# jdeschut/tunempc

Measured on AMD Instinct MI355X. Metric: stage-Hessian convexifications/sec at (nx+nu)=32, p=64, higher is better.
Workload: dtype f64

## Files before the change

include/tunempc_hip.h:

```cpp
#ifndef TUNEMPC_HIP_H
#define TUNEMPC_HIP_H

#include <stdint.h>

#ifdef __cplusplus
extern "C" {
#endif

#define TMPC_OK 0
#define TMPC_E_ARG (-1)
#define TMPC_E_UNSUPPORTED (-2)
#define TMPC_E_NOMEM (-3)
#define TMPC_E_HIP (-4)
#define TMPC_E_NODEVICE (-5)
#define TMPC_E_NOCONV (-6)

#define TMPC_STATUS_OPTIMAL 0
#define TMPC_STATUS_FEASIBLE 1
#define TMPC_STATUS_INFEASIBLE 2

#define TMPC_FLAG_NO_MFMA 1
#define TMPC_FLAG_PROFILE 2
#define TMPC_FLAG_FAST_EXIT 4

// ... 13 lines not shown
uint64_t tmpc_workspace_bytes_con(int chunk, int p, int nx, int mb, int ng, int nc);
int tmpc_create_con(tmpc_handle** out, int chunk, int p, int nx, int mb, int ng, int nc);
int tmpc_destroy(tmpc_handle* h);
int tmpc_get_chunk(tmpc_handle* h);

int tmpc_set_options(tmpc_handle* h, double tol, double center_tol, int max_iter, int center_iter, int flags);

#define TMPC_TUNE_CHORD_STEP 1
#define TMPC_TUNE_SMALL_BLOCKS 2
#define TMPC_TUNE_EIG_PRETEST 3
#define TMPC_TUNE_FUSE_FWD 4
#define TMPC_TUNE_GRAPH 5
#define TMPC_TUNE_PERSISTENT 7
#define TMPC_TUNE_LOWP_SWITCH 8
#define TMPC_LOWP_SWITCH_DEFAULT 1e-5
int tmpc_set_tuning(tmpc_handle* h, int key, double value);
int tmpc_create_ex(tmpc_handle** out, int chunk, int p, int nx, int mb, int ng, int nc, int step3, int lanes);

int tmpc_set_tight(tmpc_handle* h, int enable, double tight_tol);

int tmpc_convexify_batch_host(tmpc_handle* h, int nb, const double* A, const double* B, const double* H,
                              double* Hc, double* dHc, double* P, double* alpha, double* beta, double* kappa,
                              int32_t* status, int32_t* iters, double* info);
int tmpc_convexify_batch_device(tmpc_handle* h, int nb, const double* dA, const double* dB, const double* dH,
                                double* dHc_out, double* ddHc_out, double* dP_out, double* d_alpha, double* d_beta,
                                double* d_kappa, int32_t* d_status, int32_t* d_iters, double* d_info, void* stream);

int tmpc_convexify_eq_batch_host(tmpc_handle* h, int nb, const double* A, const double* B, const double* H, const double* G,
                                 double* Hc, double* dHc, double* P, double* Fg, double* alpha, double* beta, double* kappa,
                                 int32_t* status, int32_t* iters, double* info);
// ... 56 lines not shown
```

tunempc_amd/_lib.py:

```python
import ctypes as C
import os

import numpy as np

_HERE = os.path.dirname(os.path.abspath(__file__))
_LIB = None

INFO_STRIDE = 16
FLAG_NO_MFMA = 1
FLAG_PROFILE = 2
FLAG_FAST_EXIT = 4
STATUS_NAMES = {0: 'Optimal', 1: 'Feasible', 2: 'Infeasible'}

ARROW_LD = 32
EXPORTS = [
    'tmpc_device_count', 'tmpc_workspace_bytes', 'tmpc_workspace_bytes_eq', 'tmpc_workspace_bytes_con',
    'tmpc_create', 'tmpc_create_eq', 'tmpc_create_con', 'tmpc_destroy', 'tmpc_get_chunk', 'tmpc_set_options', 'tmpc_set_tight', 'tmpc_set_tuning', 'tmpc_create_ex',
    'tmpc_convexify_batch_host', 'tmpc_convexify_batch_device', 'tmpc_convexify_eq_batch_host', 'tmpc_convexify_step2_batch_host',
    'tmpc_convexify_con_batch_device', 'tmpc_workspace_bytes_step3', 'tmpc_create_step3', 'tmpc_convexify_step3_batch_host', 'tmpc_workspace_bytes_step3_con', 'tmpc_create_step3_con', 'tmpc_convexify_step3_con_batch_host', 'tmpc_convexify_step3_batch_device', 'tmpc_convexify_step3_con_batch_device', 'tmpc_supplement_batch_host', 'tmpc_supplement_terms_batch_host',
    'tmpc_tracking_reference_host', 'tmpc_eig_scan_host', 'tmpc_get_profile', 'tmpc_get_trace', 'tmpc_get_dual_host', 'tmpc_get_dual_con_host', 'tmpc_pack_sensitivities_host', 'tmpc_eig_clip_host',
    'tmpc_last_error', 'tmpc_version',
]
DEBUG_EXPORTS = [
    'tmpc_debug_gemm_nt', 'tmpc_debug_block_solve', 'tmpc_debug_cr_schedule', 'tmpc_debug_get_multipliers', 'tmpc_debug_get_array',
# ... 148 lines not shown
            _check(self.lib, self.lib.tmpc_create_step3_con(C.byref(self._h), int(chunk), self.p, self.nx, self.mb, self.ng, self.nc), 'tmpc_create_step3_con')
        elif self.step3:
            _check(self.lib, self.lib.tmpc_create_step3(C.byref(self._h), int(chunk), self.p, self.nx, self.mb), 'tmpc_create_step3')
        else:
            _check(self.lib, self.lib.tmpc_create_con(C.byref(self._h), int(chunk), self.p, self.nx, self.mb, self.ng, self.nc), 'tmpc_create_con')
        self.chunk = int(self.lib.tmpc_get_chunk(self._h))
        self.flags = int(flags)
        self.set_options(tol, center_tol, max_iter, center_iter, flags)

    def set_options(self, tol=None, center_tol=None, max_iter=None, center_iter=None, flags=None):
        if flags is not None:
            self.flags = int(flags)
        _check(self.lib, self.lib.tmpc_set_options(self._h, float(tol or 0.0), float(center_tol or 0.0),
                                                   int(max_iter or 0), int(center_iter or 0), self.flags), 'tmpc_set_options')

    def set_tuning(self, chord_step=None, small_blocks=None, eig_pretest=None, fuse_fwd=None, graph=None, persistent=None, lowp_switch=None):
        for key, v in ((1, chord_step), (2, small_blocks), (3, eig_pretest), (4, fuse_fwd), (5, graph), (7, persistent), (8, lowp_switch)):
            if v is not None:
                _check(self.lib, self.lib.tmpc_set_tuning(self._h, key, float(v)), 'tmpc_set_tuning')

    def set_tight(self, enable=True, tight_tol=None):
        _check(self.lib, self.lib.tmpc_set_tight(self._h, 1 if enable else 0, float(tight_tol or 0.0)), 'tmpc_set_tight')

    def close(self):
        if getattr(self, '_h', None) is not None and self._h.value:
            self.lib.tmpc_destroy(self._h)
            self._h = C.c_void_p()

    def __del__(self):
        try:
            self.close()
        except Exception:
# ... 336 lines not shown
```

tunempc_amd/csrc/tmpc_api.hip:

```cpp
#include <hip/hip_runtime.h>
#include <stdio.h>
#include <stdlib.h>
#include <new>
#include <string.h>
#include <algorithm>
#include <chrono>
#include <thread>
#include <mutex>
#include <condition_variable>
#include <functional>
#include <unistd.h>
#include <vector>

#include <string>
#include <unordered_map>

#include "../../include/tunempc_hip.h"
#include "../../include/tunempc_hip_debug.h"
#include "tmpc_common.h"
#include "tmpc_small.h"
#include "tmpc_stage.h"
#include "tmpc_schur.h"
#include "tmpc_factor.h"
#include "tmpc_cr.h"
// ... 89 lines not shown

struct tmpc_handle {
  Dims dm;
  int chunk;
  int nlanes;
  Opts opt;
  int flags;
  Lane lane[MAXL];
  void* slab;
  size_t slab_bytes;
  hipEvent_t ev_in;
  int device;
  CrSched sched;
  int* d_sched;
  int rs, mt;
  int tune_small, tune_pretest, tune_fuse, tune_graph, tune_persist;
  void* dd_slab;
  size_t dd_bytes;
  int tight;
  double tight_tol;
};

static int cr_upload(const CrSched& sc, int** out) {
  std::vector<int> flat(sc.elim);
  flat.insert(flat.end(), sc.upd.begin(), sc.upd.end());
  flat.insert(flat.end(), sc.orient.begin(), sc.orient.end());
  *out = nullptr;
  if (hipMalloc(out, flat.size() * sizeof(int)) != hipSuccess) return TMPC_E_NOMEM;
  if (hipMemcpy(*out, flat.data(), flat.size() * sizeof(int), hipMemcpyHostToDevice) != hipSuccess) { hipFree(*out); *out = nullptr; return TMPC_E_HIP; }
  return TMPC_OK;
}
// ... 289 lines not shown
static int set_lds_attrs(int device) {
  static bool done[64] = {false};
  if (device >= 0 && device < 64 && done[device]) return TMPC_OK;
  const int big = 160 * 1024;
  HIPCHK(hipFuncSetAttribute((const void*)k_stage_pre<256>, hipFuncAttributeMaxDynamicSharedMemorySize, big - 4096));
  HIPCHK(hipFuncSetAttribute((const void*)k_stage_rhs<256>, hipFuncAttributeMaxDynamicSharedMemorySize, big - 4096));
  HIPCHK(hipFuncSetAttribute((const void*)k_stage_dir<256>, hipFuncAttributeMaxDynamicSharedMemorySize, big - 4096));
  HIPCHK(hipFuncSetAttribute((const void*)k_final_stage, hipFuncAttributeMaxDynamicSharedMemorySize, big));
  HIPCHK(hipFuncSetAttribute((const void*)k_schur<0>, hipFuncAttributeMaxDynamicSharedMemorySize, big));
  HIPCHK(hipFuncSetAttribute((const void*)k_schur<1>, hipFuncAttributeMaxDynamicSharedMemorySize, big));
  HIPCHK(hipFuncSetAttribute((const void*)k_cr_potrf<true>, hipFuncAttributeMaxDynamicSharedMemorySize, big));
  HIPCHK(hipFuncSetAttribute((const void*)k_cr_potrf<false>, hipFuncAttributeMaxDynamicSharedMemorySize, big));
  HIPCHK(hipFuncSetAttribute((const void*)k_cr_trsm<true, 2>, hipFuncAttributeMaxDynamicSharedMemorySize, big));
  HIPCHK(hipFuncSetAttribute((const void*)k_cr_trsm<false, 2>, hipFuncAttributeMaxDynamicSharedMemorySize, big));
  HIPCHK(hipFuncSetAttribute((const void*)k_cr_trsm_dma, hipFuncAttributeMaxDynamicSharedMemorySize, big));
  HIPCHK(hipFuncSetAttribute((const void*)k_cr_potrf_dma, hipFuncAttributeMaxDynamicSharedMemorySize, big));
  HIPCHK(hipFuncSetAttribute((const void*)k_cr_update<true, 2>, hipFuncAttributeMaxDynamicSharedMemorySize, big));
  HIPCHK(hipFuncSetAttribute((const void*)k_cr_update<false, 2>, hipFuncAttributeMaxDynamicSharedMemorySize, big));
  HIPCHK(hipFuncSetAttribute((const void*)k_cr_fwd_diag, hipFuncAttributeMaxDynamicSharedMemorySize, big));
  HIPCHK(hipFuncSetAttribute((const void*)k_cr_fwd_off, hipFuncAttributeMaxDynamicSharedMemorySize, big));
  HIPCHK(hipFuncSetAttribute((const void*)k_cr_bwd, hipFuncAttributeMaxDynamicSharedMemorySize, big));
  HIPCHK(hipFuncSetAttribute((const void*)k_cr_small_solve, hipFuncAttributeMaxDynamicSharedMemorySize, big));
  HIPCHK(hipFuncSetAttribute((const void*)k_cr_small_factor, hipFuncAttributeMaxDynamicSharedMemorySize, big));
  HIPCHK(hipFuncSetAttribute((const void*)k_ipm_small, hipFuncAttributeMaxDynamicSharedMemorySize, big));
  HIPCHK(hipFuncSetAttribute((const void*)k_debug_gemm<true>, hipFuncAttributeMaxDynamicSharedMemorySize, big));
  HIPCHK(hipFuncSetAttribute((const void*)k_debug_gemm<false>, hipFuncAttributeMaxDynamicSharedMemorySize, big));
  HIPCHK(hipFuncSetAttribute((const void*)k_supplement, hipFuncAttributeMaxDynamicSharedMemorySize, big));
  HIPCHK(hipFuncSetAttribute((const void*)k_phi_pre<false, false>, hipFuncAttributeMaxDynamicSharedMemorySize, big));
  HIPCHK(hipFuncSetAttribute((const void*)k_phi_pre<false, true>, hipFuncAttributeMaxDynamicSharedMemorySize, big));
  HIPCHK(hipFuncSetAttribute((const void*)k_phi_pre<true, false>, hipFuncAttributeMaxDynamicSharedMemorySize, big));
// ... 12 lines not shown
  HIPCHK(hipFuncSetAttribute((const void*)k_dd_fwd_off, hipFuncAttributeMaxDynamicSharedMemorySize, big));
  HIPCHK(hipFuncSetAttribute((const void*)k_dd_bwd, hipFuncAttributeMaxDynamicSharedMemorySize, big));
  HIPCHK(hipFuncSetAttribute((const void*)k_dd_images, hipFuncAttributeMaxDynamicSharedMemorySize, big));
  HIPCHK(hipFuncSetAttribute((const void*)k_dd_schur<0>, hipFuncAttributeMaxDynamicSharedMemorySize, big));
  HIPCHK(hipFuncSetAttribute((const void*)k_dd_schur<1>, hipFuncAttributeMaxDynamicSharedMemorySize, big));
  HIPCHK(hipFuncSetAttribute((const void*)k_dd_schur<0, true>, hipFuncAttributeMaxDynamicSharedMemorySize, big));
  HIPCHK(hipFuncSetAttribute((const void*)k_dd_schur<1, true>, hipFuncAttributeMaxDynamicSharedMemorySize, big));
  HIPCHK(hipFuncSetAttribute((const void*)k_dd_polish_pre, hipFuncAttributeMaxDynamicSharedMemorySize, big - 4096));
  HIPCHK(hipFuncSetAttribute((const void*)k_polish_step, hipFuncAttributeMaxDynamicSharedMemorySize, big - 4096));
  if (device >= 0 && device < 64) done[device] = true;
  return TMPC_OK;
}

static unsigned cr_grid(long items) { return (unsigned)((items + 7) / 8 * 8); }
constexpr int DF_NO_SMALL = 2;
constexpr int DF_LOWP = 8;
constexpr int DF_NO_DMA = 4;

static bool cr_small_levels(const Dims& dm, const CrSched& sc, CrLevs* out) {
  if ((dm.flags & DF_NO_SMALL) || dm.dp != 16 || (dm.flags & 1) || dm.p > CRS_PMAX || (int)sc.lev.size() > CRS_MAXLEV) return false;
  if (out) {
    out->n = (int)sc.lev.size();
    for (int l = 0; l < out->n; ++l) { out->v[4 * l] = sc.lev[l].eoff; out->v[4 * l + 1] = sc.lev[l].nelim; out->v[4 * l + 2] = sc.lev[l].uoff; out->v[4 * l + 3] = sc.lev[l].nupd; }
  }
  return true;
}

static void cr_factor(const WS& w, const Dims& dm, const CrSched& sc, const int* d_sched, const int* alist, int count, hipStream_t st,
                      int rs_opt, int mt_opt, std::vector<hipEvent_t>* kev = nullptr, int* nkev = nullptr, int fuse_fwd1 = 0, int nlowp = 0) {
  const CrDev cd = cr_dev(sc, d_sched, alist);
  int ke = 0;
// ... 26 lines not shown
      hipLaunchKernelGGL(k_cr_potrf_dma, dim3(cr_grid((long)count * lv.nelim)), dim3(256), (size_t)potrf_dma_lds_doubles() * sizeof(double), st, w, dm, cd, lv.eoff, lv.nelim, count);
    else if (mf) hipLaunchKernelGGL(k_cr_potrf<true>, dim3(cr_grid((long)count * lv.nelim)), dim3(256), factor_lds(), st, w, dm, cd, lv.eoff, lv.nelim, count);
    else hipLaunchKernelGGL(k_cr_potrf<false>, dim3(cr_grid((long)count * lv.nelim)), dim3(256), factor_lds(), st, w, dm, cd, lv.eoff, lv.nelim, count);
    mark(0);
    if (fuse_fwd1) hipLaunchKernelGGL(k_cr_fwd_diag, dim3(cr_grid((long)count * lv.nelim)), dim3(256), solve_lds(dm), st, w, dm, cd, lv.eoff, lv.nelim, count, 1);
    if (lv.nupd == 0) { mark(1); mark(1); mark(2); mark(2); mark(3); mark(3); continue; }
    const long work64 = (long)count * lv.nelim * 2 * nt64;
    const int rs = rs_opt > 0 ? rs_opt : (work64 >= 16384 ? 128 : 64);
    const int mt = mt_opt > 0 ? mt_opt : 64;
    const int nstrip = (dm.dp + rs - 1) / rs, nm = (dm.dp + mt - 1) / mt;
    const long it_trsm = (long)count * lv.nelim * 2 * nstrip;
    const long it_upd = (long)count * ((long)lv.nupd * (nm * (nm + 1) / 2) + (long)lv.nelim * nm * nm);
    mark(1);
    if (mf && use_dma && dm.nt <= TRR_NT) {
      const size_t trsm_lds = (size_t)trd_lds_doubles() * sizeof(double);
      hipLaunchKernelGGL(k_cr_trsm_dma, dim3(cr_grid((long)count * lv.nelim * 2 * nt64)), dim3(256), trsm_lds, st, w, dm, cd, lv.eoff, lv.nelim, count);
    }
    else if (mf) hipLaunchKernelGGL((k_cr_trsm<true, 2>), dim3(cr_grid(it_trsm)), dim3(256), factor_lds(), st, w, dm, cd, lv.eoff, lv.nelim, count, rs);
    else hipLaunchKernelGGL((k_cr_trsm<false, 2>), dim3(cr_grid(it_trsm)), dim3(256), factor_lds(), st, w, dm, cd, lv.eoff, lv.nelim, count, rs);
    mark(1); mark(2);
    if (mf && use_dma) {
      const int nm64 = (dm.dp + 63) / 64;
      const long it_dma = (long)count * ((long)lv.nupd * (nm64 * (nm64 + 1) / 2) + (long)lv.nelim * nm64 * nm64);
      if (nlowp < count)
        hipLaunchKernelGGL(k_cr_update_dma, dim3(cr_grid(it_dma)), dim3(256), (size_t)dma_lds_doubles<UPD_DMA_DEPTH>() * sizeof(double), st, w, dm, cd, lv.eoff, lv.nelim, lv.uoff, lv.nupd, count, fuse_fwd1);
      mark(2); mark(3);
      if (nlowp > 0)
        hipLaunchKernelGGL(k_cr_update_dma_f32, dim3(cr_grid(it_dma)), dim3(256), (size_t)UPD_DMA_DEPTH * DMA_SLAB * sizeof(double), st, w, dm, cd, lv.eoff, lv.nelim, lv.uoff, lv.nupd, count);
      mark(3);
    }
    else if (mf) { hipLaunchKernelGGL((k_cr_update<true, 2>), dim3(cr_grid(it_upd)), dim3(256), factor_lds(), st, w, dm, cd, lv.eoff, lv.nelim, lv.uoff, lv.nupd, count, mt); mark(2); mark(3); mark(3); }
// ... 95 lines not shown
    if (hipMalloc(&ln->big_scr, (size_t)h->dm.B * dm.p * BIG_SCR * dm.n * dm.n * sizeof(double)) != hipSuccess) { snprintf(g_err, sizeof(g_err), "hipMalloc of the generic-stage scratch failed"); return TMPC_E_NOMEM; }
    ln->ws.bscr = (double*)ln->big_scr;
  }
  WS wall = ln->ws;
  wall.A = dA; wall.Bm = dB; wall.H = dH; wall.G = dG; wall.ncnt = dncnt; wall.rho = rho;
  wall.cr_orient = h->d_sched + h->sched.elim.size() + h->sched.upd.size();
  WS w = wall;
  w.A = nullptr; w.Bm = nullptr; w.H = nullptr;
  int* alist = wall.alist;
  int* flist = wall.flist;
  wall.alist = nullptr;
  Opts o = h->opt;
  o.tight = 0; o.tight_tol = 0.0;
  o.fast_exit = (h->flags & TMPC_FLAG_FAST_EXIT) ? 1 : 0;
  if ((h->flags & (TMPC_FLAG_NO_MFMA | TMPC_DEBUG_FLAG_NO_DMA)) || !w.O32 || t3 || dm.dp <= 64 || dm.nt > TRR_NT) o.lowp_switch = 0.0;
  if (o.lowp_switch > 0.0) {
    dm.flags |= DF_LOWP;
    if (ln->o32_dp != 0 && ln->o32_dp != dm.dp) HIPCHK(hipMemsetAsync(w.O32, 0, 2 * (size_t)h->dm.B * h->dm.p * h->dm.dp * ((h->dm.dp + 31) & ~31) * sizeof(float), st));
    ln->o32_dp = dm.dp;
  }
  WS wf = w; wf.alist = flist;
  const int BPall = nb * dm.p;
  const bool prof = (h->flags & TMPC_FLAG_PROFILE) != 0;
  bool use_graph = h->tune_graph && dm.dp <= 64 && !(h->flags & (TMPC_FLAG_PROFILE | TMPC_DEBUG_FLAG_STOP_ASSEMBLED)) && st == ln->st;
  const int reg_max = (h->flags & TMPC_DEBUG_FLAG_NO_LIFT) ? 0 : REG_MAX;
  HIPCHK(hipMemsetAsync(w.active, 0, 5 * sizeof(int), st));
  HIPCHK(hipMemsetAsync(w.trace, 0, (size_t)nb * TRACE_LEN * TRACE_W * sizeof(double), st));
  const size_t big_lds = (size_t)BIG_EIG_LDS * sizeof(double);
  if (big) hipLaunchKernelGGL(kb_init_stage, dim3(BPall), dim3(256), big_lds, st, wall, dm);
  else hipLaunchKernelGGL(k_init_stage, dim3(BPall), dim3(64), slots_bytes(2), st, wall, dm);
  {
    WS wi = wall; wi.alist = alist;
    hipLaunchKernelGGL(k_init_prob, dim3(nb), dim3(64), 0, st, wi, dm);
  }
  hipLaunchKernelGGL(k_init_state, dim3(BPall), dim3(64), 0, st, wall, dm);
  if (eq) hipLaunchKernelGGL(k_phi_init, dim3(BPall), dim3(64), 0, st, wall, dm);
  if (t3) hipLaunchKernelGGL(k_t3_init, dim3(BPall), dim3(64), 0, st, wall, dm);
  int cnt[5] = {0, 0, 0, 0, 0};
  HIPCHK(hipMemcpyAsync(cnt, w.active, 5 * sizeof(int), hipMemcpyDeviceToHost, st));
  HIPCHK(hipStreamSynchronize(st));
  int active = cnt[0], nfac = cnt[0], nlowp = cnt[4];
  const int cap = o.max_iter + o.center_iter * (MUT_BACKOFF_MAX + 1) + 2;
  int it = 0;
  {
    CrLevs plv;
    const bool pays = h->tune_persist >= 2 || dm.p <= 8 || active * h->nlanes >= 96;
    const bool persist = h->tune_persist && pays && !eq && !t3 && !big && dm.dp == 16 && dm.n <= PK_NMAX && !h->tight && !prof &&
                         !(h->flags & TMPC_DEBUG_FLAG_STOP_ASSEMBLED) && cr_small_levels(dm, h->sched, &plv);
// ... 308 lines not shown
    chunk = (int)std::max<uint64_t>(1, std::min<uint64_t>(512, fit));
  }
  tmpc_handle* h = new (std::nothrow) tmpc_handle();
  if (!h) return TMPC_E_NOMEM;
  h->slab = nullptr; h->d_sched = nullptr; h->ev_in = nullptr; h->dd_slab = nullptr; h->dd_bytes = 0; h->tight = 0; h->tight_tol = 0x1p-37;
  if (hipGetDevice(&h->device) != hipSuccess) { delete h; return TMPC_E_HIP; }
  int nl = (make_dims(1, p, nx, mb, ng, nc, step3).dp <= 64 && chunk >= 2) ? 2 : 1;
  if (lanes >= 1) nl = std::min(lanes, MAXL);
  nl = std::max(1, std::min(nl, chunk));
  h->nlanes = nl;
  const int cap = (chunk + nl - 1) / nl;
  h->chunk = cap * nl;
  h->dm = make_dims(cap, p, nx, mb, ng, nc, step3);
  h->sched = cr_build(p);
  h->rs = 0; h->mt = 0;
  h->tune_small = 1; h->tune_pretest = 1; h->tune_fuse = 1; h->tune_graph = 1; h->tune_persist = 1;
  h->opt.tol = 0x1p-25; h->opt.center_tol = 1e-9; h->opt.max_iter = 50; h->opt.center_iter = 12;
  h->opt.fast_exit = 0;
  h->opt.lowp_switch = TMPC_LOWP_SWITCH_DEFAULT;
  h->opt.chord_step = 10.0;
  h->flags = 0;
  WS tmp;
  const size_t lane_bytes = carve(tmp, h->dm, nullptr, nullptr);
  h->slab_bytes = lane_bytes * nl;
  if (hipMalloc(&h->slab, h->slab_bytes) != hipSuccess) {
    snprintf(g_err, sizeof(g_err), "hipMalloc(%zu bytes) failed", h->slab_bytes);
    delete h;
    return TMPC_E_NOMEM;
  }
  int rc = cr_upload(h->sched, &h->d_sched);
  bool ok = (rc == TMPC_OK) && hipEventCreateWithFlags(&h->ev_in, hipEventDisableTiming) == hipSuccess;
// ... 50 lines not shown
  h->flags = flags;
  return TMPC_OK;
}


int tmpc_set_tuning(tmpc_handle* h, int key, double value) {
  if (!h) return TMPC_E_ARG;
  switch (key) {
    case TMPC_TUNE_CHORD_STEP: if (!(value >= 0.0)) return TMPC_E_ARG; h->opt.chord_step = value; return TMPC_OK;
    case TMPC_TUNE_LOWP_SWITCH: if (!(value >= 0.0)) return TMPC_E_ARG; h->opt.lowp_switch = value; return TMPC_OK;
    case TMPC_TUNE_SMALL_BLOCKS: h->tune_small = value != 0.0; return TMPC_OK;
    case TMPC_TUNE_EIG_PRETEST: h->tune_pretest = value != 0.0; return TMPC_OK;
    case TMPC_TUNE_FUSE_FWD: h->tune_fuse = value != 0.0; return TMPC_OK;
    case TMPC_TUNE_GRAPH: h->tune_graph = value != 0.0; return TMPC_OK;
    case TMPC_TUNE_PERSISTENT: if (!(value >= 0.0 && value <= 2.0)) return TMPC_E_ARG; h->tune_persist = (int)value; return TMPC_OK;
    default: snprintf(g_err, sizeof(g_err), "tmpc_set_tuning: unknown key %d", key); return TMPC_E_ARG;
  }
}

int tmpc_set_tight(tmpc_handle* h, int enable, double tight_tol) {
  if (!h) return TMPC_E_ARG;
  if (!enable) { h->tight = 0; return TMPC_OK; }
  if (h->dm.nT > 0) { snprintf(g_err, sizeof(g_err), "tmpc_set_tight: Steps 1 and 2 only (no Step 3 handles)"); return TMPC_E_UNSUPPORTED; }
  if (h->dm.nr > 0 && (size_t)dd_aug_lds_doubles(h->dm.nr, h->dm.n, h->dm.nx) * sizeof(double) > 160 * 1024) {
    snprintf(g_err, sizeof(g_err), "tmpc_set_tight: %d rows per stage at nx = %d, nx + mb = %d: their double-double vectors do not fit the LDS (rows * (2 n + 2 nx) <= 4040)", h->dm.nr, h->dm.nx, h->dm.n);
    return TMPC_E_UNSUPPORTED;
  }
  if ((size_t)dd_solve_lds_doubles(h->dm.dp) * sizeof(double) > 160 * 1024) {
    snprintf(g_err, sizeof(g_err), "tmpc_set_tight: Schur blocks of %d do not fit the LDS image of the double-double substitution kernels (nx <= 51)", h->dm.dp);
    return TMPC_E_UNSUPPORTED;
// ... 704 lines not shown
```

tunempc_amd/csrc/tmpc_common.h:

```cpp
#pragma once
#include <hip/hip_runtime.h>
#include <stdint.h>

namespace tmpc {

#ifdef TMPC_CYCLE_PROF
__device__ unsigned long long g_prof[64];
__device__ int g_prof_cls;
#define TMPC_T(i) { if (blockIdx.x == 0 && threadIdx.x == 0) { const unsigned long long t_ = __builtin_readcyclecounter(); g_prof[(g_prof_cls & 7) * 8 + (i)] += t_ - tprev_; tprev_ = t_; } }
#define TMPC_T0() unsigned long long tprev_ = __builtin_readcyclecounter();
#define TMPC_TC(c, i) { if (blockIdx.x == 0 && threadIdx.x == 0) { const unsigned long long t_ = __builtin_readcyclecounter(); g_prof[(c) * 8 + (i)] += t_ - tprevc_; tprevc_ = t_; } }
#define TMPC_TC0() unsigned long long tprevc_ = __builtin_readcyclecounter();
#else
#define TMPC_TC(c, i)
#define TMPC_TC0()
#define TMPC_T(i)
#define TMPC_T0()
#endif



constexpr double ALPHA_MIN = 1e-8;
constexpr int TRACE_LEN = 80, TRACE_W = 10;
constexpr int TB = 64;
// ... 15 lines not shown
enum { IPM_OPTIMAL = 0, IPM_INACCURATE = 1, IPM_MAXITER = 2, IPM_FAST_EXIT = 3, IPM_TIGHT_FALLBACK = 4 };
enum { ST_OPTIMAL = 0, ST_FEASIBLE = 1, ST_INFEASIBLE = 2 };

enum {
  Q_XS = 0, Q_RD2, Q_S2, Q_TRX2, Q_HBY, Q_TRPSI, Q_TRPHI2, Q_HBPHI,
  Q_TRT2, Q_HBG,
  Q_MINX, Q_MINS, Q_DXS, Q_XDS, Q_DXDS, Q_DP2, Q_P2,
  Q_MINEIG, Q_MINABS, Q_MAXABS, Q_MAXEIG, Q_CHOLBAD, Q_DH2, Q_M2,
  Q_RPHI2, Q_NCONE,
  NPART = 26
};

typedef double double2_t __attribute__((ext_vector_type(2)));
typedef double double4_t __attribute__((ext_vector_type(4)));
typedef float float4_t __attribute__((ext_vector_type(4)));
enum { KF_XXX = 0, KF_SIXX, KF_KX, KF_KS, KF_FX, KF_FS, KF_PER_LMI = 6 };
enum { ADJ_G = 0, ADJ_PSI, ADJ_PHI, NADJ = 3 };

struct Dims {
  int B;
  int p;
  int nx, mb;
  int n;
  int d;
  int dp;
  int nt;
  int flags;
  int ng;
  int nr;
  int nz;
  int constr;
  int nT;
};
constexpr int NGM = 31;
constexpr int NCM = 31;
constexpr int NRM = NGM + NCM, NZM = NRM + 2;
constexpr int NRS = 32, NZS = NRS + 2;
constexpr int NAM = 31;
constexpr int AEL = NAM + 1, AE = AEL * AEL;

struct Opts {
  double tol;
  double center_tol;
  int max_iter;
  int center_iter;
  double chord_step;
  int tight;
  double tight_tol;
// ... 80 lines not shown
```

tunempc_amd/csrc/tmpc_cr.h:

```cpp
#pragma once
#include <climits>
#include <vector>

#include "tmpc_common.h"
#include "tmpc_factor.h"
#include "tmpc_gemm_dma.h"

namespace tmpc {

constexpr int CR_EW = 8;
constexpr int CR_UW = 8;
enum { CE_NODE = 0, CE_NA, CE_NB, CE_EA, CE_EB, CE_FILL, CE_FX, CE_FACC };
enum { CU_NODE = 0, CU_E0, CU_S0, CU_E1, CU_S1 };

struct CrLevel { int eoff, nelim, uoff, nupd; };
struct CrSched {
  int p = 0;
  int prep = 0;
  std::vector<int> orient;
  std::vector<int> elim, upd;
  std::vector<CrLevel> lev;
};

static inline CrSched cr_build(int p) {
// ... 475 lines not shown
  const int per = 2 * nst;
  const int it = cr_item(count * nelim * per);
  if (it < 0) return;
  extern __shared__ __attribute__((aligned(16))) double lds[];
  const int g = it / per, r = it - g * per;
  const int b = cr.alist[g / nelim];
  const int* er = cr.elim + (size_t)(eoff + g % nelim) * CR_EW;
  const int which = r / nst, strip = r - which * nst;
  const int slot = which ? er[CE_EB] : er[CE_EA];
  if (slot < 0) return;
  const int node = er[CE_NODE];
  const double* Dk = w.D + ((size_t)b * dm.p + node) * (size_t)dp * dp;
  const double* Li = w.Linv + ((size_t)b * dm.p + node) * dm.nt * TB * TB;
  const int r0 = strip * 64;
  const bool lp = cr_lowp(w, b);
  const int ld32 = cr_ld32(dm);
  trd_strip<false>(cr_edge(w, dm, b, slot) + (size_t)r0 * dp, Dk, Li, (dp - r0 < 64) ? dp - r0 : 64, dm.nt, dp, it, lds,
                   lp ? cr_edge32(w, dm, b, slot) + (size_t)r0 * ld32 : nullptr, ld32);
}

constexpr int potrf_dma_lds_doubles() { return FACT_LDS_DOUBLES > trd_lds_doubles() ? FACT_LDS_DOUBLES : trd_lds_doubles(); }
__global__ void __launch_bounds__(256, 2) k_cr_potrf_dma(WS w, Dims dm, CrDev cr, int eoff, int nelim, int count) {
  const int it = cr_item(count * nelim);
  if (it < 0) return;
  extern __shared__ __attribute__((aligned(16))) double lds[];
  const int b = cr.alist[it / nelim];
  const int* er = cr.elim + (size_t)(eoff + it % nelim) * CR_EW;
  const int node = er[CE_NODE], dp = dm.dp;
  double* Dk = w.D + ((size_t)b * dm.p + node) * (size_t)dp * dp;
  double* Li = w.Linv + ((size_t)b * dm.p + node) * dm.nt * TB * TB;
  const double* dref = w.Ddiag + ((size_t)b * dm.p + node) * dp;
  double* stat = lds + FACT_LDS_DOUBLES - 8;
  if (threadIdx.x == 0) { stat[0] = 0.0; stat[1] = 1.0; }
// ... 255 lines not shown
```

tunempc_amd/csrc/tmpc_stage.h:

```cpp
#pragma once
#include "tmpc_common.h"
#include "tmpc_small.h"

namespace tmpc {

__device__ __forceinline__ int stage_id4(const WS& w, const Dims& dm) {
  if (!w.alist) return blockIdx.x;
  const int sb = blockIdx.x >> 2, bi = sb / dm.p;
  return ((w.alist[bi] * dm.p + (sb - bi * dm.p)) << 2) | (blockIdx.x & 3);
}

#define TMPC_STAGE_PROLOGUE                                     \
  const int sid = stage_id(w, dm);                              \
  const int b = sid / dm.p;                                     \
  const int k = sid - b * dm.p;                                 \
  const int lane = threadIdx.x;                                 \
  const int n = dm.n, nx = dm.nx;                               \
  const int nn = n * n, nxx = nx * nx;                          \
  (void)k; (void)nn; (void)nxx;                                 \
  extern __shared__ __attribute__((aligned(16))) double sm[];

#ifdef TMPC_EIG_DEBUG
__device__ int g_eig_dbg[4]; __device__ double g_eig_dbgv[8];
#endif
// ... 30 lines not shown
  lo = wave_min(lo); hi = wave_max(hi); amin = wave_min(amin); amax = wave_max(amax);
  if (lane == 0) {
    double* q = w.part + (size_t)sid * NPART;
    q[Q_MINEIG] = lo; q[Q_MAXEIG] = hi; q[Q_MINABS] = amin; q[Q_MAXABS] = amax;
  }
  const int mb = dm.mb;
  double* Vg = w.V + (size_t)sid * nx * n;
  const double* Ag = w.A + (size_t)sid * nxx;
  const double* Bg = w.Bm + (size_t)sid * nx * mb;
  for (int e = lane; e < nx * n; e += 64) {
    int i, j; ediv(e, n, i, j);
    Vg[e] = (j < nx) ? Ag[i * nx + j] : Bg[i * mb + (j - nx)];
  }
}

__global__ void __launch_bounds__(64) k_init_prob(WS w, Dims dm) {
  const int b = blockIdx.x, lane = threadIdx.x;
  double lo = 1e300, amin = 1e10 , amax = 0.0;
  for (int k = lane; k < dm.p; k += 64) {
    const double* q = w.part + (size_t)(b * dm.p + k) * NPART;
    lo = fmin(lo, q[Q_MINEIG]); amin = fmin(amin, q[Q_MINABS]); amax = fmax(amax, q[Q_MAXABS]);
  }
  lo = wave_min(lo); amin = wave_min(amin); amax = wave_max(amax);
  if (lane == 0) {
    double* pr = w.prob + (size_t)b * PS;
    int* ip = w.iprob + (size_t)b * IS;
    for (int i = 0; i < PS; ++i) pr[i] = 0.0;
    for (int i = 0; i < IS; ++i) ip[i] = 0;
    const double s = 1.0 / amin, sbeta = amax / amin;
    pr[P_S] = s; pr[P_SBETA] = sbeta; pr[P_MINEIG_H] = lo;
    pr[P_TAU] = 2.0; pr[P_ALPHA] = 1.0 / sbeta; pr[P_S0] = 1.0 / sbeta; pr[P_X0] = 1.0 / (double)(dm.p * dm.n);
    pr[P_MUT] = -1.0; pr[P_PREVSTEPN] = -1.0; pr[P_STEPN] = 1e300; pr[P_MINPIV] = 1.0;
    const int early = (lo > 0.0) ? 1 : 0;
    ip[I_EARLY] = early;
    ip[I_PHASE] = early ? PH_DONE : PH_MAIN;
    ip[I_IPMSTATUS] = early ? IPM_OPTIMAL : IPM_MAXITER;
    if (!early) { const int slot = atomicAdd(w.active, 1); w.alist[slot] = b; w.flist[slot] = b; }
    if (!early && (dm.flags & 8) && w.O32) { ip[I_LOWP] = 1; atomicAdd(w.active + 4, 1); }
  }
}

__global__ void __launch_bounds__(64) k_init_state(WS w, Dims dm) {
  TMPC_STAGE_PROLOGUE
  const double* pr = w.prob + (size_t)b * PS;
  const double s = pr[P_S], tau = pr[P_TAU], alpha = pr[P_ALPHA];
  const double x0 = 1.0 / (double)(dm.p * n);
  double* Hb = w.Hb + (size_t)sid * nn;
  for (int e = lane; e < nn; e += 64) {
    int i, j; ediv(e, n, i, j);
    const double hb = s * Hb[e];
    Hb[e] = hb;
    const double dg = (i == j) ? 1.0 : 0.0;
    w.S1[(size_t)sid * nn + e] = dg;
// ... 210 lines not shown
```

Baseline: 11830.

## Add fp32 MFMA triangular-solve path for low-precision cyclic-reduction batches

Adds a new fp32 DMA-pipelined triangular-solve kernel that uses f32 MFMA and writes straight into the fp32 edge buffers. Batches in low-precision mode are routed to it, while the fp64 trsm kernel skips them. The aim is to cut the cost of the fp64 trsm for those batches. It also changes the low-precision start condition, clamping the switch threshold to at least 16x the tolerance and gating initial low-precision mode on the barrier parameter, which can change which problems use low precision and the iteration behaviour.

```diff
diff --git a/include/tunempc_hip.h b/include/tunempc_hip.h
--- a/include/tunempc_hip.h
+++ b/include/tunempc_hip.h
@@ -51,6 +51,7 @@
 #define TMPC_TUNE_PERSISTENT 7
 #define TMPC_TUNE_LOWP_SWITCH 8
 #define TMPC_LOWP_SWITCH_DEFAULT 1e-5
+#define TMPC_TUNE_LOWP_TRSM 9
 int tmpc_set_tuning(tmpc_handle* h, int key, double value);
 int tmpc_create_ex(tmpc_handle** out, int chunk, int p, int nx, int mb, int ng, int nc, int step3, int lanes);
 
diff --git a/tunempc_amd/_lib.py b/tunempc_amd/_lib.py
--- a/tunempc_amd/_lib.py
+++ b/tunempc_amd/_lib.py
@@ -186,8 +186,8 @@
         _check(self.lib, self.lib.tmpc_set_options(self._h, float(tol or 0.0), float(center_tol or 0.0),
                                                    int(max_iter or 0), int(center_iter or 0), self.flags), 'tmpc_set_options')
 
-    def set_tuning(self, chord_step=None, small_blocks=None, eig_pretest=None, fuse_fwd=None, graph=None, persistent=None, lowp_switch=None):
-        for key, v in ((1, chord_step), (2, small_blocks), (3, eig_pretest), (4, fuse_fwd), (5, graph), (7, persistent), (8, lowp_switch)):
+    def set_tuning(self, chord_step=None, small_blocks=None, eig_pretest=None, fuse_fwd=None, graph=None, persistent=None, lowp_switch=None, lowp_trsm=None):
+        for key, v in ((1, chord_step), (2, small_blocks), (3, eig_pretest), (4, fuse_fwd), (5, graph), (7, persistent), (8, lowp_switch), (9, lowp_trsm)):
             if v is not None:
                 _check(self.lib, self.lib.tmpc_set_tuning(self._h, key, float(v)), 'tmpc_set_tuning')
 
diff --git a/tunempc_amd/csrc/tmpc_api.hip b/tunempc_amd/csrc/tmpc_api.hip
--- a/tunempc_amd/csrc/tmpc_api.hip
+++ b/tunempc_amd/csrc/tmpc_api.hip
@@ -127,7 +127,7 @@
   CrSched sched;
   int* d_sched;
   int rs, mt;
-  int tune_small, tune_pretest, tune_fuse, tune_graph, tune_persist;
+  int tune_small, tune_pretest, tune_fuse, tune_graph, tune_persist, tune_lowp_trsm;
   void* dd_slab;
   size_t dd_bytes;
   int tight;
@@ -447,6 +447,7 @@
   HIPCHK(hipFuncSetAttribute((const void*)k_cr_trsm<true, 2>, hipFuncAttributeMaxDynamicSharedMemorySize, big));
   HIPCHK(hipFuncSetAttribute((const void*)k_cr_trsm<false, 2>, hipFuncAttributeMaxDynamicSharedMemorySize, big));
   HIPCHK(hipFuncSetAttribute((const void*)k_cr_trsm_dma, hipFuncAttributeMaxDynamicSharedMemorySize, big));
+  HIPCHK(hipFuncSetAttribute((const void*)k_cr_trsm_dma_f32, hipFuncAttributeMaxDynamicSharedMemorySize, big));
   HIPCHK(hipFuncSetAttribute((const void*)k_cr_potrf_dma, hipFuncAttributeMaxDynamicSharedMemorySize, big));
   HIPCHK(hipFuncSetAttribute((const void*)k_cr_update<true, 2>, hipFuncAttributeMaxDynamicSharedMemorySize, big));
   HIPCHK(hipFuncSetAttribute((const void*)k_cr_update<false, 2>, hipFuncAttributeMaxDynamicSharedMemorySize, big));
@@ -489,7 +490,6 @@
 
 static unsigned cr_grid(long items) { return (unsigned)((items + 7) / 8 * 8); }
 constexpr int DF_NO_SMALL = 2;
-constexpr int DF_LOWP = 8;
 constexpr int DF_NO_DMA = 4;
 
 static bool cr_small_levels(const Dims& dm, const CrSched& sc, CrLevs* out) {
@@ -546,7 +546,11 @@
     mark(1);
     if (mf && use_dma && dm.nt <= TRR_NT) {
       const size_t trsm_lds = (size_t)trd_lds_doubles() * sizeof(double);
-      hipLaunchKernelGGL(k_cr_trsm_dma, dim3(cr_grid((long)count * lv.nelim * 2 * nt64)), dim3(256), trsm_lds, st, w, dm, cd, lv.eoff, lv.nelim, count);
+      const bool trsm32 = (dm.flags & DF_LOWP_TRSM) != 0;
+      if (!trsm32 || nlowp < count)
+        hipLaunchKernelGGL(k_cr_trsm_dma, dim3(cr_grid((long)count * lv.nelim * 2 * nt64)), dim3(256), trsm_lds, st, w, dm, cd, lv.eoff, lv.nelim, count);
+      if (trsm32 && nlowp > 0)
+        hipLaunchKernelGGL(k_cr_trsm_dma_f32, dim3(cr_grid((long)count * lv.nelim * 2 * nt64)), dim3(256), (size_t)trf_lds_doubles() * sizeof(double), st, w, dm, cd, lv.eoff, lv.nelim, count);
     }
     else if (mf) hipLaunchKernelGGL((k_cr_trsm<true, 2>), dim3(cr_grid(it_trsm)), dim3(256), factor_lds(), st, w, dm, cd, lv.eoff, lv.nelim, count, rs);
     else hipLaunchKernelGGL((k_cr_trsm<false, 2>), dim3(cr_grid(it_trsm)), dim3(256), factor_lds(), st, w, dm, cd, lv.eoff, lv.nelim, count, rs);
@@ -672,8 +676,9 @@
   o.tight = 0; o.tight_tol = 0.0;
   o.fast_exit = (h->flags & TMPC_FLAG_FAST_EXIT) ? 1 : 0;
   if ((h->flags & (TMPC_FLAG_NO_MFMA | TMPC_DEBUG_FLAG_NO_DMA)) || !w.O32 || t3 || dm.dp <= 64 || dm.nt > TRR_NT) o.lowp_switch = 0.0;
+  if (o.lowp_switch > 0.0) o.lowp_switch = fmax(o.lowp_switch, 16.0 * o.tol);
   if (o.lowp_switch > 0.0) {
-    dm.flags |= DF_LOWP;
+    dm.flags |= DF_LOWP | (h->tune_lowp_trsm ? DF_LOWP_TRSM : 0);
     if (ln->o32_dp != 0 && ln->o32_dp != dm.dp) HIPCHK(hipMemsetAsync(w.O32, 0, 2 * (size_t)h->dm.B * h->dm.p * h->dm.dp * ((h->dm.dp + 31) & ~31) * sizeof(float), st));
     ln->o32_dp = dm.dp;
   }
@@ -689,7 +694,7 @@
   else hipLaunchKernelGGL(k_init_stage, dim3(BPall), dim3(64), slots_bytes(2), st, wall, dm);
   {
     WS wi = wall; wi.alist = alist;
-    hipLaunchKernelGGL(k_init_prob, dim3(nb), dim3(64), 0, st, wi, dm);
+    hipLaunchKernelGGL(k_init_prob, dim3(nb), dim3(64), 0, st, wi, dm, o.lowp_switch);
   }
   hipLaunchKernelGGL(k_init_state, dim3(BPall), dim3(64), 0, st, wall, dm);
   if (eq) hipLaunchKernelGGL(k_phi_init, dim3(BPall), dim3(64), 0, st, wall, dm);
@@ -1028,7 +1033,7 @@
   h->dm = make_dims(cap, p, nx, mb, ng, nc, step3);
   h->sched = cr_build(p);
   h->rs = 0; h->mt = 0;
-  h->tune_small = 1; h->tune_pretest = 1; h->tune_fuse = 1; h->tune_graph = 1; h->tune_persist = 1;
+  h->tune_small = 1; h->tune_pretest = 1; h->tune_fuse = 1; h->tune_graph = 1; h->tune_persist = 1; h->tune_lowp_trsm = 1;
   h->opt.tol = 0x1p-25; h->opt.center_tol = 1e-9; h->opt.max_iter = 50; h->opt.center_iter = 12;
   h->opt.fast_exit = 0;
   h->opt.lowp_switch = TMPC_LOWP_SWITCH_DEFAULT;
@@ -1109,6 +1114,7 @@
     case TMPC_TUNE_FUSE_FWD: h->tune_fuse = value != 0.0; return TMPC_OK;
     case TMPC_TUNE_GRAPH: h->tune_graph = value != 0.0; return TMPC_OK;
     case TMPC_TUNE_PERSISTENT: if (!(value >= 0.0 && value <= 2.0)) return TMPC_E_ARG; h->tune_persist = (int)value; return TMPC_OK;
+    case TMPC_TUNE_LOWP_TRSM: h->tune_lowp_trsm = value != 0.0; return TMPC_OK;
     default: snprintf(g_err, sizeof(g_err), "tmpc_set_tuning: unknown key %d", key); return TMPC_E_ARG;
   }
 }
diff --git a/tunempc_amd/csrc/tmpc_common.h b/tunempc_amd/csrc/tmpc_common.h
--- a/tunempc_amd/csrc/tmpc_common.h
+++ b/tunempc_amd/csrc/tmpc_common.h
@@ -53,6 +53,7 @@
 typedef double double2_t __attribute__((ext_vector_type(2)));
 typedef double double4_t __attribute__((ext_vector_type(4)));
 typedef float float4_t __attribute__((ext_vector_type(4)));
+typedef float float2_t __attribute__((ext_vector_type(2)));
 enum { KF_XXX = 0, KF_SIXX, KF_KX, KF_KS, KF_FX, KF_FS, KF_PER_LMI = 6 };
 enum { ADJ_G = 0, ADJ_PSI, ADJ_PHI, NADJ = 3 };
 
@@ -71,6 +72,8 @@
   int constr;
   int nT;
 };
+constexpr int DF_LOWP = 8;
+constexpr int DF_LOWP_TRSM = 16;
 constexpr int NGM = 31;
 constexpr int NCM = 31;
 constexpr int NRM = NGM + NCM, NZM = NRM + 2;
diff --git a/tunempc_amd/csrc/tmpc_cr.h b/tunempc_amd/csrc/tmpc_cr.h
--- a/tunempc_amd/csrc/tmpc_cr.h
+++ b/tunempc_amd/csrc/tmpc_cr.h
@@ -513,9 +513,257 @@
   const double* Li = w.Linv + ((size_t)b * dm.p + node) * dm.nt * TB * TB;
   const int r0 = strip * 64;
   const bool lp = cr_lowp(w, b);
+  if (lp && (dm.flags & DF_LOWP_TRSM)) return;
   const int ld32 = cr_ld32(dm);
   trd_strip<false>(cr_edge(w, dm, b, slot) + (size_t)r0 * dp, Dk, Li, (dp - r0 < 64) ? dp - r0 : 64, dm.nt, dp, it, lds,
                    lp ? cr_edge32(w, dm, b, slot) + (size_t)r0 * ld32 : nullptr, ld32);
+}
+
+constexpr int trf_lds_doubles() { return 2048 + TRD_DEPTH * 2048; }
+__device__ __forceinline__ void trf_strip(const double* X, const double* Dk, const double* Li, int rows, int nt, int dp, int it, double* lds, float* X32, int ld32) {
+  constexpr int ASL = 64 * 16, DP = TRD_DEPTH;
+  const int tid = threadIdx.x;
+  const int lane = tid & 63, wv = __builtin_amdgcn_readfirstlane(tid >> 6);
+  const int ws = (wv + it) & 3, wc0 = ws * 16;
+  const int fk = lane >> 4, fr = lane & 15;
+  const int i1 = (rows + 15) >> 4;
+  const int nlast = nt - 1, nbl = (dp - 64 * nlast < 64) ? dp - 64 * nlast : 64, ncl = nbl >> 4;
+  const int ntd = nt;
+  const bool rw = ws < i1;
+  float* At = (float*)lds;
+  double* Bs = lds + 2048;
+  unsigned voT[2], voL[2];
+#pragma unroll
+  for (int h = 0; h < 2; ++h) {
+    const int row = wv * 16 + 8 * h + (lane >> 3), c = lane & 7;
+    voT[h] = (unsigned)(row * TB + 2 * (c ^ dma_sw(row))) * 8u;
+    voL[h] = (unsigned)(row * dp + 2 * (c ^ dma_sw(row))) * 8u;
+  }
+  int of[2];
+#pragma unroll
+  for (int hh = 0; hh < 2; ++hh) of[hh] = fr * 16 + 2 * ((4 * hh + fk) ^ dma_sw(fr));
+  const int asw = (fr >> 1) & 3, ofa = fr * 16 + 4 * (fk ^ asw);
+  const int opa0 = 4 * ((2 * fk) & 3 ^ asw) + 2 * (fk >> 1), opa1 = 4 * ((2 * fk + 1) & 3 ^ asw) + 2 * (fk >> 1);
+  float4_t acc0[4], acc1[4], acc2[4], acc3[4];
+  int vmtot = 0, vmk0 = 0, vmk1 = 0, vmk2 = 0;
+#define TRF_NB(T) ((dp - 64 * (T) < 64) ? dp - 64 * (T) : 64)
+#define TRF_LOAD_C(I, SET)                                                                                  \
+  {                                                                                                         \
+    const bool on_ = wc0 < TRF_NB(I);                                                                       \
+    _Pragma("unroll") for (int i = 0; i < 4; ++i) {                                                          \
+      double2_t u0 = (double2_t){0.0, 0.0}, u1 = u0;                                                        \
+      if (on_ && i < i1) {                                                                                  \
+        gcptr2 cp = (gcptr2)(X + (size_t)(16 * i + fr) * dp + 64 * (I) + wc0 + 4 * fk);                     \
+        u0 = cp[0]; u1 = cp[1];                                                                             \
+      }                                                                                                     \
+      SET[i] = (float4_t){(float)-u0[0], (float)-u0[1], (float)-u1[0], (float)-u1[1]};                      \
+    }                                                                                                       \
+    if (on_) vmtot += 2 * i1;                                                                               \
+  }
+#define TRF_LOAD_R(I, NC, SET)                                                                              \
+  {                                                                                                         \
+    _Pragma("unroll") for (int c = 0; c < 4; ++c) {                                                          \
+      double2_t u0 = (double2_t){0.0, 0.0}, u1 = u0;                                                        \
+      if (rw && c < (NC)) {                                                                                 \
+        gcptr2 cp = (gcptr2)(X + (size_t)(wc0 + fr) * dp + 64 * (I) + 16 * c + 4 * fk);                     \
+        u0 = cp[0]; u1 = cp[1];                                                                             \
+      }                                                                                                     \
+      SET[c] = (float4_t){(float)-u0[0], (float)-u0[1], (float)-u1[0], (float)-u1[1]};                      \
+    }                                                                                                       \
+    if (rw) vmtot += 2 * (NC);                                                                              \
+  }
+#define TRF_STORE_R(I, NC, SET)                                                                             \
+  if (rw) {                                                                                                 \
+    typedef float4_t __attribute__((address_space(1)))* gptr4;                                              \
+    _Pragma("unroll") for (int c = 0; c < 4; ++c)                                                            \
+      if (c < (NC)) *(gptr4)(X32 + (size_t)(wc0 + fr) * ld32 + 64 * (I) + 16 * c + 4 * fk) = SET[c];        \
+    vmtot += (NC);                                                                                          \
+  }
+#define TRF_PARK_C(SET)                                                                        \
+  {                                                                                                         \
+    _Pragma("unroll") for (int i = 0; i < 4; ++i) {                                                          \
+      float* q = At + ws * ASL + (16 * i + fr) * 16;                                                        \
+      *(float2_t*)(q + opa0) = (float2_t){-SET[i][0], -SET[i][1]};                                           \
+      *(float2_t*)(q + opa1) = (float2_t){-SET[i][2], -SET[i][3]};                                           \
+    }                                                                                                       \
+  }
+#define TRF_PARK_R(NC, SET, SG)                                                                             \
+  if (rw) {                                                                                                 \
+    _Pragma("unroll") for (int c = 0; c < 4; ++c) {                                                          \
+      if (c < (NC)) {                                                                                       \
+        float* q = At + c * ASL + (wc0 + fr) * 16;                                                          \
+        *(float2_t*)(q + opa0) = (float2_t){SG SET[c][0], SG SET[c][1]};                                     \
+        *(float2_t*)(q + opa1) = (float2_t){SG SET[c][2], SG SET[c][3]};                                     \
+      }                                                                                                     \
+    }                                                                                                       \
+  }
+#define TRF_ZERO(SET) { _Pragma("unroll") for (int i = 0; i < 4; ++i) SET[i] = (float4_t){0.f, 0.f, 0.f, 0.f}; }
+  int ii = 0, ij = 0, is = 0, nissued = 0, ndone = 0;
+#define TRF_ISSUE()                                                       \
+  {                                                                                                         \
+    if (ii < ntd) {                                                                                         \
+      double* dst_ = Bs + (nissued % DP) * 2048 + wv * 256;                                                 \
+      const int nsl_ = (ij == ii) ? (TRF_NB(ii) >> 4) : 4;                                                  \
+      const bool two_ = 2 * is + 1 < nsl_;                                                                  \
+      if (ij == ii) {                                                                                       \
+        const int nb_ = TRF_NB(ii);                                                                         \
+        const __amdgpu_buffer_rsrc_t rs_ = __builtin_amdgcn_make_buffer_rsrc((void*)(Li + (size_t)ii * TB * TB), 0, (int)(((unsigned)(nb_ - 1) * TB + (unsigned)nb_) * 8u), 0x00020000); \
+        __builtin_amdgcn_raw_ptr_buffer_load_lds(rs_, (lds_vptr)(dst_), 16, voT[0], is * 256, 0, 0);        \
+        __builtin_amdgcn_raw_ptr_buffer_load_lds(rs_, (lds_vptr)(dst_ + 128), 16, voT[1], is * 256, 0, 0);  \
+        if (two_) {                                                                                         \
+          __builtin_amdgcn_raw_ptr_buffer_load_lds(rs_, (lds_vptr)(dst_ + 1024), 16, voT[0], is * 256 + 128, 0, 0);       \
+          __builtin_amdgcn_raw_ptr_buffer_load_lds(rs_, (lds_vptr)(dst_ + 1024 + 128), 16, voT[1], is * 256 + 128, 0, 0); \
+        }                                                                                                   \
+      } else {                                                                                              \
+        const int nb_ = TRF_NB(ij);                                                                         \
+        const __amdgpu_buffer_rsrc_t rs_ = __builtin_amdgcn_make_buffer_rsrc((void*)(Dk + (size_t)(64 * ij) * dp + 64 * ii), 0, (int)(((unsigned)(nb_ - 1) * (unsigned)dp + 64u) * 8u), 0x00020000); \
+        __builtin_amdgcn_raw_ptr_buffer_load_lds(rs_, (lds_vptr)(dst_), 16, voL[0], is * 256, 0, 0);        \
+        __builtin_amdgcn_raw_ptr_buffer_load_lds(rs_, (lds_vptr)(dst_ + 128), 16, voL[1], is * 256, 0, 0);  \
+        __builtin_amdgcn_raw_ptr_buffer_load_lds(rs_, (lds_vptr)(dst_ + 1024), 16, voL[0], is * 256 + 128, 0, 0);         \
+        __builtin_amdgcn_raw_ptr_buffer_load_lds(rs_, (lds_vptr)(dst_ + 1024 + 128), 16, voL[1], is * 256 + 128, 0, 0);   \
+      }                                                                                                     \
+      vmtot += (ij == ii && !two_) ? 2 : 4;                                                                 \
+      { const int k_ = nissued % DP; if (k_ == 0) vmk0 = vmtot; else if (k_ == 1) vmk1 = vmtot; else vmk2 = vmtot; }  \
+      ++nissued;                                                                                            \
+      if (++is == ((nsl_ + 1) >> 1)) { is = 0; if (++ij >= ntd) { ++ii; ij = ii; } }                        \
+    }                                                                                                       \
+  }
+#define TRF_MMA_C(TGT, AS, BS)                                                                              \
+  {                                                                                                         \
+    float4_t a_[4];                                                                                          \
+    _Pragma("unroll") for (int i = 0; i < 4; ++i) a_[i] = *(const float4_t*)((AS) + i * 256 + ofa);         \
+    _Pragma("unroll") for (int hh = 0; hh < 2; ++hh) {                                                      \
+      const double2_t b_ = *(const double2_t*)((BS) + wc0 * 16 + of[hh]);                                   \
+      _Pragma("unroll") for (int e = 0; e < 2; ++e) {                                                        \
+        const float bf_ = (float)b_[e];                                                                      \
+        _Pragma("unroll") for (int i = 0; i < 4; ++i)                                                        \
+          TGT[i] = __builtin_amdgcn_mfma_f32_16x16x4f32(bf_, a_[i][2 * hh + e], TGT[i], 0, 0, 0);           \
+      }                                                                                                     \
+    }                                                                                                       \
+  }
+#define TRF_MMA_R(TGT, AS, BS, C0, NC)                                                                      \
+  {                                                                                                         \
+    const float4_t a_ = *(const float4_t*)((AS) + wc0 * 16 + ofa);                                          \
+    _Pragma("unroll") for (int hh = 0; hh < 2; ++hh) {                                                      \
+      double2_t b_[4];                                                                                       \
+      _Pragma("unroll") for (int c = 0; c < 4; ++c)                                                          \
+        if (c >= (C0) && c < (NC)) b_[c] = *(const double2_t*)((BS) + c * 256 + of[hh]);                    \
+      _Pragma("unroll") for (int e = 0; e < 2; ++e) {                                                        \
+        _Pragma("unroll") for (int c = 0; c < 4; ++c)                                                        \
+          if (c >= (C0) && c < (NC)) TGT[c] = __builtin_amdgcn_mfma_f32_16x16x4f32((float)b_[c][e], a_[2 * hh + e], TGT[c], 0, 0, 0); \
+      }                                                                                                     \
+    }                                                                                                       \
+  }
+#define TRF_STEP_C(TGT) { TRF_MMA_C(TGT, A0, Bc) TRF_MMA_C(TGT, A0 + ASL, Bc + 1024) }
+#define TRF_STEP_D0(TGT) { TRF_MMA_R(TGT, At, Bc, 0, 4) TRF_MMA_R(TGT, At + ASL, Bc + 1024, 1, 4) }
+#define TRF_STEP_D1(TGT) { TRF_MMA_R(TGT, At + 2 * ASL, Bc, 2, 4) TRF_MMA_R(TGT, At + 3 * ASL, Bc + 1024, 3, 4) }
+#define TRF_STEP_RL(N) { TRF_MMA_R(acc0, A0, Bc, 0, N) TRF_MMA_R(acc0, A0 + ASL, Bc + 1024, 0, N) }
+
+  __syncthreads();
+  TRF_ISSUE()
+  if (DP > 2) TRF_ISSUE()
+  TRF_LOAD_C(0, acc0)
+  if (nt > 2) TRF_LOAD_C(1, acc1) else TRF_ZERO(acc1)
+  if (nt > 3) TRF_LOAD_C(2, acc2) else TRF_ZERO(acc2)
+  if (nt > 4) TRF_LOAD_C(3, acc3) else TRF_ZERO(acc3)
+  TRF_PARK_C(acc0)
+  TRF_ZERO(acc0)
+#define TRF_STEP_BEGIN()                                                                                    \
+    { const int k_ = ndone % DP; vm_wait_le(vmtot - (k_ == 0 ? vmk0 : k_ == 1 ? vmk1 : vmk2)); }            \
+    __builtin_amdgcn_s_barrier();                                                                           \
+    TRF_ISSUE()                                                                                             \
+    const double* Bc = Bs + (ndone % DP) * 2048;                                                            \
+    ++ndone;
+#define TRF_PAIR_C(TGT)                                                                                     \
+  _Pragma("unroll 1") for (int cs = 0; cs < 2; ++cs) {                                                      \
+    TRF_STEP_BEGIN()                                                                                        \
+    const float* A0 = At + 2 * cs * ASL;                                                                    \
+    TRF_STEP_C(TGT)                                                                                         \
+  }
+#define TRF_PAIR_RL(N)                                                                                      \
+  _Pragma("unroll 1") for (int cs = 0; cs < 2; ++cs) {                                                      \
+    TRF_STEP_BEGIN()                                                                                        \
+    const float* A0 = At + 2 * cs * ASL;                                                                    \
+    if (rw) TRF_STEP_RL(N)                                                                                  \
+  }
+#define TRF_DIAG(TGT)                                                                                       \
+  {                                                                                                         \
+    { TRF_STEP_BEGIN() if (rw) TRF_STEP_D0(TGT) }                                                           \
+    { TRF_STEP_BEGIN() if (rw) TRF_STEP_D1(TGT) }                                                           \
+    TRF_STORE_R(ci, 4, TGT)                                                                                 \
+    if (ci + 1 < nt) {                                                                                      \
+      __builtin_amdgcn_s_barrier();                                        \
+      TRF_PARK_R(4, TGT, +)                                                                                 \
+    }                                                                                                       \
+  }
+  for (int ci = 0; ci < ntd; ++ci) {
+    const int nci = TRF_NB(ci) >> 4;
+    if (nci == 4) {
+      if (ci == 0 || ci == nlast) TRF_DIAG(acc0) else if (ci == 1) TRF_DIAG(acc1) else if (ci == 2) TRF_DIAG(acc2) else TRF_DIAG(acc3)
+    } else {
+      for (int cs = 0; cs < ((nci + 1) >> 1); ++cs) {
+        TRF_STEP_BEGIN()
+        const float* A0 = At + 2 * cs * ASL;
+        if (rw) {
+          TRF_MMA_R(acc0, A0, Bc, 2 * cs, nci)
+          if (2 * cs + 1 < nci) TRF_MMA_R(acc0, A0 + ASL, Bc + 1024, 2 * cs + 1, nci)
+        }
+      }
+      TRF_STORE_R(ci, nci, acc0)
+    }
+    if (ci == 0 && nt > 1) TRF_LOAD_R(nlast, ncl, acc0)
+    if (ci + 1 >= nt) break;
+    if (ci < 1 && 1 < nlast) TRF_PAIR_C(acc1)
+    if (ci < 2 && 2 < nlast) TRF_PAIR_C(acc2)
+    if (ci < 3 && 3 < nlast) TRF_PAIR_C(acc3)
+    if (ncl == 3) TRF_PAIR_RL(3) else if (ncl == 4) TRF_PAIR_RL(4) else if (ncl == 2) TRF_PAIR_RL(2) else TRF_PAIR_RL(1)
+    const int t = ci + 1;
+    __builtin_amdgcn_s_barrier();
+    if (t == nlast) { TRF_PARK_R(ncl, acc0, -) TRF_ZERO(acc0) }
+    else if (t == 1) { TRF_PARK_C(acc1) TRF_ZERO(acc1) }
+    else if (t == 2) { TRF_PARK_C(acc2) TRF_ZERO(acc2) }
+    else { TRF_PARK_C(acc3) TRF_ZERO(acc3) }
+  }
+#undef TRF_DIAG
+#undef TRF_PAIR_RL
+#undef TRF_PAIR_C
+#undef TRF_STEP_BEGIN
+#undef TRF_STEP_RL
+#undef TRF_STEP_D1
+#undef TRF_STEP_D0
+#undef TRF_STEP_C
+#undef TRF_MMA_R
+#undef TRF_MMA_C
+#undef TRF_ISSUE
+#undef TRF_ZERO
+#undef TRF_PARK_R
+#undef TRF_PARK_C
+#undef TRF_STORE_R
+#undef TRF_LOAD_R
+#undef TRF_LOAD_C
+#undef TRF_NB
+}
+
+__global__ void __launch_bounds__(256, 2) k_cr_trsm_dma_f32(WS w, Dims dm, CrDev cr, int eoff, int nelim, int count) {
+  const int dp = dm.dp;
+  const int nst = (dp + 63) / 64;
+  const int per = 2 * nst;
+  const int it = cr_item(count * nelim * per);
+  if (it < 0) return;
+  extern __shared__ __attribute__((aligned(16))) double lds[];
+  const int g = it / per, r = it - g * per;
+  const int b = cr.alist[g / nelim];
+  if (!cr_lowp(w, b)) return;
+  const int* er = cr.elim + (size_t)(eoff + g % nelim) * CR_EW;
+  const int which = r / nst, strip = r - which * nst;
+  const int slot = which ? er[CE_EB] : er[CE_EA];
+  if (slot < 0) return;
+  const int node = er[CE_NODE];
+  const double* Dk = w.D + ((size_t)b * dm.p + node) * (size_t)dp * dp;
+  const double* Li = w.Linv + ((size_t)b * dm.p + node) * dm.nt * TB * TB;
+  const int r0 = strip * 64;
+  const int ld32 = cr_ld32(dm);
+  trf_strip(cr_edge(w, dm, b, slot) + (size_t)r0 * dp, Dk, Li, (dp - r0 < 64) ? dp - r0 : 64, dm.nt, dp, it, lds, cr_edge32(w, dm, b, slot) + (size_t)r0 * ld32, ld32);
 }
 
 constexpr int potrf_dma_lds_doubles() { return FACT_LDS_DOUBLES > trd_lds_doubles() ? FACT_LDS_DOUBLES : trd_lds_doubles(); }
diff --git a/tunempc_amd/csrc/tmpc_stage.h b/tunempc_amd/csrc/tmpc_stage.h
--- a/tunempc_amd/csrc/tmpc_stage.h
+++ b/tunempc_amd/csrc/tmpc_stage.h
@@ -68,7 +68,7 @@
   }
 }
 
-__global__ void __launch_bounds__(64) k_init_prob(WS w, Dims dm) {
+__global__ void __launch_bounds__(64) k_init_prob(WS w, Dims dm, double lowp_switch) {
   const int b = blockIdx.x, lane = threadIdx.x;
   double lo = 1e300, amin = 1e10 , amax = 0.0;
   for (int k = lane; k < dm.p; k += 64) {
@@ -90,7 +90,7 @@
     ip[I_PHASE] = early ? PH_DONE : PH_MAIN;
     ip[I_IPMSTATUS] = early ? IPM_OPTIMAL : IPM_MAXITER;
     if (!early) { const int slot = atomicAdd(w.active, 1); w.alist[slot] = b; w.flist[slot] = b; }
-    if (!early && (dm.flags & 8) && w.O32) { ip[I_LOWP] = 1; atomicAdd(w.active + 4, 1); }
+    if (!early && (dm.flags & DF_LOWP) && w.O32 && 2.0 / (double)(2 * dm.p * dm.n + 1) > lowp_switch * fmax(1.0, fabs(pr[P_TAU]))) { ip[I_LOWP] = 1; atomicAdd(w.active + 4, 1); }
   }
 }
 
```

After: 12130, median of 6. 1.03x the previous value.
